# Fireflies-17/Speech-Inpainting

Hardware: AMD Instinct MI355X
Metric: real-time factor (audio-sec/wall-sec) per GPU, 4 s clips @16 kHz, 200 ms mask (higher is better)
Workload: dtype encoder GEMMs and attention products: bf16 MFMA, fp32 accumulate (softmax, LayerNorm, head, arg-max in fp32); vocoder: fp16 MFMA (operands rounded to fp16, saturating), fp32 accumulate, activations stored as fp16; 1 GPU; BASELINE configs[1]: batch=32 x 4 s clips per GPU, 200 ms mask, HuBERT-base + HiFi-GAN V1; step = masked log-mel front-end -> encoder -> arg-max/splice -> vocoder on resident raw clips; global_batch=32, clip_samples=64000, mask_frames=10, parallelism=utterance-sharded x1

## Files before the change

### include/si_hip.h

```cpp
#ifndef SI_HIP_H
#define SI_HIP_H

#include <stddef.h>
#include <stdint.h>

#ifdef __cplusplus
extern "C" {
#endif

#define SI_ABI_VERSION 3

enum {
    SI_OK = 0,
    SI_EINVAL = -1,
    SI_ENOMEM = -2,
    SI_EHIP = -3,
    SI_ESTATE = -4,
    SI_EWEIGHTS = -5
};

enum {
    SI_MATH_F32 = 0,
    SI_MATH_BF16 = 1,
    SI_MATH_BF16X3 = 2,
// ... 241 lines not shown
typedef struct si_profile_entry {
    char name[48];
    int32_t launches;
    int32_t reserved;
    double ms;
    double flops;
    double bytes;
} si_profile_entry;
int si_profile_start(si_ctx* ctx, int max_launches);
int si_profile_filter(si_ctx* ctx, const char* family);
int si_profile_stop(si_ctx* ctx, si_profile_entry* out, int capacity, int* count);

int si_debug_capture(si_ctx* ctx, const char* name, float* dst, long capacity);
long si_debug_size(si_ctx* ctx, const char* name);

#ifdef __cplusplus
}
#endif
#endif
```

### speech_inpainting_amd/csrc/api.hip

```cpp
#include <cmath>
#include <cstdarg>
#include <cstdio>
#include <cstdlib>
#include <cstring>
#include <map>
#include <sstream>
#include <string>
#include <vector>

#include "common.h"

namespace {

struct HostTensor {
    const float* data = nullptr;
    std::vector<long> shape;
    long numel() const { long n = 1; for (long d : shape) n *= d; return n; }
};

struct GemmW {
    size_t w = 0, w_lo = 0, bias = 0;
    int Cin = 0, N = 0, Npad = 0, ntaps = 0, groups = 1, math = 0;
    bool has_bias = false;
};
// ... 33 lines not shown
    std::string prof_filter;
    std::vector<std::string> prof_names;
    std::vector<ProfRec> prof_recs;
    std::vector<hipEvent_t> prof_pool;
    size_t prof_used = 0;
    int prof_open = -1;
    int num_cus = 0;
    std::map<const void*, size_t> dyn_lds;
    bool opt_voc_opready = true, opt_voc_res16 = true, opt_enc_opready = true, opt_att_bf16 = true, opt_enc_lingemm = true;
    bool opt_enc_posconv = true;
    int opt_ln_fuse = 1;
    int opt_voc_upsgemm = 1;
    int opt_ffn_pad = 64;
    int opt_gemmcu = 1;
    int opt_voc_chain = 1;
    int opt_voc_fuse = 1;
    char* fe_dev = nullptr;
    size_t fe_dft = 0, fe_hann = 0, fe_basis = 0, fe_lo = 0, fe_hi = 0;
    std::vector<int32_t> vl_host;
    static constexpr int VL_SLOTS = 4;
    int32_t* vl_pin[VL_SLOTS] = {nullptr, nullptr, nullptr, nullptr};
    size_t vl_pin_ints[VL_SLOTS] = {0, 0, 0, 0};
    hipEvent_t vl_ev[VL_SLOTS] = {nullptr, nullptr, nullptr, nullptr};
    int vl_next = 0;
    float* km_cnorm = nullptr;
    int km_cnorm_cap = 0;
};

static char g_create_err[512] = "";

// ... 486 lines not shown
    EncDims e = enc_dims(d, N);
    size_t cmax = 0;
    for (int i = 0; i < d.num_conv; ++i) cmax = std::max(cmax, (size_t)e.L[i + 1] * d.conv_dim[i]);
    const size_t BT = (size_t)B * std::max(e.T, 1);
    size_t f = 2 * (size_t)B * cmax + BT * d.conv_dim[d.num_conv - 1] + BT * d.hidden_size * 3 + BT * 3 * d.hidden_size + BT * d.intermediate_size +
               (size_t)B * d.conv_dim[0] * 2 + BT * 2;
    const size_t h16 = (BT * d.conv_dim[d.num_conv - 1] + 2 * BT * d.hidden_size + BT * (d.intermediate_size + 128)) * 2;
    return f * 4 + h16 + (size_t)B * 16 + (size_t)B * 4 + si_conv0_partials_bytes(B, N) + 41 * 256 +
           align_up((size_t)(SI_MAX_CONV + 3) * (B + 1) * 4, 256);
}

int vocoder_chunk(const si_model_desc& d, int B) { int c = d.vocoder_chunk > 0 ? d.vocoder_chunk : 32; return std::min(c, std::max(B, 1)); }

long voc_tout(int Tm, int stretch) { return stretch ? (long)std::floor((double)Tm * (441.0 / 256.0)) : Tm; }

size_t vocoder_ws_bytes(const si_ctx* ctx, int B, int Tm, int stretch) {
    const si_model_desc& d = ctx->d;
    const int Bc = vocoder_chunk(d, B);
    const long Tout = voc_tout(Tm, stretch);
    size_t lc_max = (size_t)Tout * d.up_initial_channel;
    long L = Tout; int c = d.up_initial_channel;
    for (int i = 0; i < d.num_ups; ++i) { L *= d.up_rates[i]; c = stage_channels(ctx, i); lc_max = std::max(lc_max, (size_t)L * c); }
    const size_t f = (size_t)Bc * Tout * ctx->lay.mel_ld + 9 * (size_t)Bc * lc_max;
    return f * 4 + 32 * 256 + align_up((size_t)(2 * SI_MAX_UPS + 3) * B * 4, 256);
}

TapGemmParams gemm_params(const si_ctx* ctx, const GemmW& G) {
    TapGemmParams p{};
    p.w = ctx->wdev + G.w;
    p.w_lo = G.math == SI_MATH_BF16X3 ? ctx->wdev + G.w_lo : nullptr;
    p.bias = G.has_bias ? reinterpret_cast<const float*>(ctx->wdev + G.bias) : nullptr;
    p.Cin = G.Cin; p.N = G.N; p.Npad = G.Npad; p.ntaps = G.ntaps; p.groups = G.groups;
    p.stride = 1; p.dil = 1; p.pad = 0; p.pro_slope = 1.f; p.act = SI_ACT_NONE; p.alpha = 1.f; p.accumulate = 0;
    p.out16_slope = 1.f;
    p.nseg = 1;
    return p;
}

struct UpsGeom { int u, pad; long Lout; int M; };
// ... 56 lines not shown
    if (!out) return si_fail(nullptr, SI_EINVAL, "si_create: out is NULL");
    *out = nullptr;
    int rc = check_desc(nullptr, desc);
    if (rc) return rc;
    int ndev = 0;
    if (hipGetDeviceCount(&ndev) != hipSuccess || device_id < 0 || device_id >= ndev)
        return si_fail(nullptr, SI_EHIP, "si_create: device %d not available (%d HIP devices visible)", device_id, ndev);
    si_ctx* ctx = new si_ctx();
    ctx->device = device_id;
    ctx->d = *desc;
    auto env_flag = [](const char* name) { const char* v = getenv(name); return v ? atoi(v) != 0 : true; };
    ctx->opt_voc_opready = env_flag("SI_VOC_OPREADY");
    ctx->opt_voc_res16 = env_flag("SI_VOC_RES16");
    ctx->opt_voc_fuse = getenv("SI_VOC_FUSE") ? atoi(getenv("SI_VOC_FUSE")) : 1;
    ctx->opt_voc_chain = getenv("SI_VOC_CHAIN") ? atoi(getenv("SI_VOC_CHAIN")) : 1;
    ctx->opt_enc_opready = env_flag("SI_ENC_OPREADY");
    ctx->opt_att_bf16 = env_flag("SI_ATT_BF16");
    ctx->opt_enc_lingemm = env_flag("SI_ENC_LINGEMM");
    ctx->opt_enc_posconv = env_flag("SI_ENC_POSCONV");
    ctx->opt_gemmcu = getenv("SI_ENC_GEMMCU") ? atoi(getenv("SI_ENC_GEMMCU")) : 1;
    ctx->opt_ln_fuse = getenv("SI_ENC_LNFUSE") ? atoi(getenv("SI_ENC_LNFUSE")) : 1;
    ctx->opt_voc_upsgemm = getenv("SI_VOC_UPSGEMM") ? atoi(getenv("SI_VOC_UPSGEMM")) : 1;
    ctx->opt_ffn_pad = getenv("SI_ENC_FFNPAD") ? std::min(128, std::max(0, atoi(getenv("SI_ENC_FFNPAD")) / 8 * 8)) : 64;
    plan_layout(ctx);
    *out = ctx;
    return SI_OK;
}

void si_destroy(si_ctx* ctx) {
    if (!ctx) return;
// ... 688 lines not shown
                    const UpsGeom g = ups_geom(d, i, Lb);
                    t[(size_t)(2 + i) * B + b] = (int32_t)g.Lout;
                    t[(size_t)(2 + d.num_ups + i) * B + b] = g.M;
                    Lb = g.Lout;
                }
            }
            return SI_OK;
        })) return trc;
        SI_HIP_CHECK(hipMemsetAsync(wav_out, 0, (size_t)B * Lwav * sizeof(float), st));
    }
    float* ext_ws = W.floats((size_t)Bc_max * Tout * Ly.mel_ld);
    float* buf_ws[6];
    unsigned short* h16_ws[6];
    for (auto& b : buf_ws) b = W.floats((size_t)Bc_max * lc_max);
    for (auto& b : h16_ws) b = reinterpret_cast<unsigned short*>(W.bytes((size_t)Bc_max * lc_max * 2));
    const bool opr = ctx->opt_voc_opready && (d.vocoder_math == SI_MATH_BF16 || d.vocoder_math == SI_MATH_F16);
    const bool r16 = opr && ctx->opt_voc_res16 && d.vocoder_math == SI_MATH_F16;
    const int fuse_mask = ctx->opt_voc_fuse == 1 ? ~0 : ctx->opt_voc_fuse;
    if (!W.ok) return si_fail(ctx, SI_ENOMEM, "internal: vocoder workspace carve exceeded its own estimate");
    const int nk = d.num_rb;
    static const char* upn[] = {"ups0", "ups1", "ups2", "ups3", "ups4", "ups5", "ups6", "ups7"};
    static const char* stn[] = {"stage0", "stage1", "stage2", "stage3", "stage4", "stage5", "stage6", "stage7"};

    auto run = [&](int b0, int Bc, float* ext, float* const* buf, unsigned short* const* h16, hipStream_t st) -> int {
        int rc;
        auto tap16 = [&](const void* src, long n, const char* fmt, int a = 0, int b = 0, int c = 0) -> int {
            return (r16 && !ctx->dbg_capture.empty()) ? si_tap(ctx, st, {src, n, 2}, fmt, a, b, c) : SI_OK;
        };
        auto tap32 = [&](TapSrc s, const char* fmt, int a = 0, int b = 0, int c = 0) -> int {
            return (!r16 && !ctx->dbg_capture.empty()) ? si_tap(ctx, st, s, fmt, a, b, c) : SI_OK;
        };
        const int32_t* dTm = vl ? tab.dev + b0 : nullptr;
        auto dLs = [&](int sidx) -> const int32_t* { return vl ? tab.dev + (size_t)(1 + sidx) * B + b0 : nullptr; };
        auto hLs = [&](int sidx) -> const int32_t* { return vl ? tab.host + (size_t)(1 + sidx) * B + b0 : nullptr; };
        auto rows_of = [&](const int32_t* h, long uniform) { if (!h) return (double)Bc * uniform; double r = 0; for (int b = 0; b < Bc; ++b) r += h[b]; return r; };
        auto stage_conv = [&](const GemmW& G, int sidx, long L, int ld_in, int cin, int dil) {
            TapGemmParams p = gemm_params(ctx, G);
            p.nseg = Bc; p.Lin = (int)L; p.M = (int)L; p.ldx = ld_in; p.x_seg_stride = L * ld_in;
            p.dil = dil; p.pad = dil * (G.ntaps - 1) / 2; p.ldo = G.N; p.o_seg_stride = L * G.N; p.olimit = p.o_seg_stride;
// ... 54 lines not shown
                p.pro_slope = act_in ? 1.f : in_slope;
                const int urc = act_in ? si_launch_gemmcu_tc(ctx, p, st, true) : 1;
                if (urc < 0) return urc;
                if (urc > 0 && (rc = si_launch_tapgemm(ctx, G.math, p, st))) return rc;
            }
            const long nst = (long)Bc * Lo * cout;
            if (!r16 && (rc = si_tap(ctx, st, {U, nst}, upn[i]))) return rc;
            if ((rc = tap16(U16, nst, "ups%d.f16", i))) return rc;
            const bool act_next = ups_takes_activated(i + 1, Lo, cout);
            struct BlockOut { float alpha; int accumulate; bool copy16; float slope16; };
            auto block_out = [&](int j, bool last) {
                const bool completes = last && j == nk - 1;
                return BlockOut{last ? 1.0f / nk : 1.f, last && j > 0, r16 || !last || (completes && i + 1 < d.num_ups),
                                (r16 && !(completes && act_next)) ? 1.f : 0.1f};
            };
            for (int j = 0; j < nk; ++j) {
                const ResW& R = Ly.rbs[(size_t)i * nk + j];
                const int rk = d.rb_kernels[j];
                const float* y = U;
                const unsigned short* y16 = U16;
                const BlockOut whole = block_out(j, true);
                if (r16 && d.resblock_type != 2 && (fuse_mask & cout) && ctx->opt_voc_chain && d.num_dil == 3 && whole.slope16 == 1.f) {
                    ResChainParams cp{};
                    cp.y16 = U16; cp.out16 = xs16; cp.B = Bc; cp.L = (int)Lo; cp.k = rk; cp.alpha = whole.alpha; cp.accumulate = whole.accumulate;
                    cp.lens = dLs(i + 1); cp.lens_host = hLs(i + 1);
                    for (int n = 0; n < 3; ++n) {
                        const TapGemmParams w1 = gemm_params(ctx, R.c1[n]), w2 = gemm_params(ctx, R.c2[n]);
                        cp.w1[n] = static_cast<const unsigned short*>(w1.w); cp.w2[n] = static_cast<const unsigned short*>(w2.w);
                        cp.b1[n] = w1.bias; cp.b2[n] = w2.bias; cp.dil[n] = d.rb_dilations[j][n];
                    }
                    const int crc = si_launch_reschain(ctx, cout, cp, st);
                    if (crc < 0) return crc;
                    if (crc == 0) {
                        if ((rc = tap16(xs16, nst, "stage%d.rb%d.p%d.f16", i, j, d.num_dil - 1))) return rc;
                        continue;
                    }
                }
                for (int n = 0; n < d.num_dil; ++n) {
                    const int dl = d.rb_dilations[j][n];
                    const bool last = (n == d.num_dil - 1);
                    float* ynext = last ? xs : buf[4 + (n & 1)];
                    unsigned short* ynext16 = last ? xs16 : h16[4 + (n & 1)];
                    const BlockOut o = block_out(j, last);
                    auto residual_conv = [&](const GemmW& G, int dil, float slope, const float* in, const unsigned short* in16) {
                        TapGemmParams q = stage_conv(G, i + 1, Lo, cout, cout, dil);
                        q.x = in; q.out = ynext; q.res = y; q.pro_slope = slope;
                        if (opr) {
                            q.x = nullptr; q.x16 = in16;
                            if (r16) { q.res = nullptr; q.res16 = y16; q.out = nullptr; }
                            if (o.copy16) { q.out16 = ynext16; q.out16_slope = o.slope16; }
                        }
                        q.alpha = o.alpha; q.accumulate = o.accumulate; q.acc16 = r16 && o.accumulate;
                        return si_launch_tapgemm(ctx, G.math, q, st);
                    };
                    if (d.resblock_type == 2) {
                        if ((rc = residual_conv(R.c1[n], dl, in_slope, y, y16))) return rc;
                    } else {
// ... 21 lines not shown
                    y16 = ynext16;
                }
            }
            if (!r16 && (rc = si_tap(ctx, st, {xs, nst}, stn[i]))) return rc;
            if ((rc = tap16(xs16, nst, "stage%d.f16", i))) return rc;
            std::swap(x, xs);
            std::swap(x16, xs16);
            Lc = Lo; c = cout; act_in = act_next;
        }
        return si_launch_conv_post(ctx, x, wf(ctx, Ly.post_w), wf(ctx, Ly.post_b), Bc, (int)Lc, c, 7, wav_out + (size_t)b0 * Lwav, st,
                                   r16 ? x16 : nullptr, dLs(d.num_ups), hLs(d.num_ups));
    };

    for (int b0 = 0; b0 < B; b0 += Bc_max) {
        const int Bc = std::min(Bc_max, B - b0);
        if (int rc = run(b0, Bc, ext_ws, buf_ws, h16_ws, st)) return rc;
    }
    return SI_OK;
}

}

namespace {

constexpr int FE_NFFT = 1024, FE_HOP = 441, FE_PAD = 312, FE_NMEL = 80, FE_SR = 22050, FE_NBIN = FE_NFFT / 2 + 1;
constexpr double FE_FMIN = 0.0, FE_FMAX = 8000.0;
constexpr int FE_KC = 528, FE_KS = 512;
constexpr int FE_FRAME = FE_KC + FE_KS;
constexpr int FE_IMOFF = 516;
constexpr int FE_LDSPEC = 1032;

// ... 387 lines not shown
```

### speech_inpainting_amd/csrc/common.h

```cpp
#pragma once
#include <hip/hip_runtime.h>
#include <stdint.h>

#include "../../include/si_hip.h"

#define SI_HIP_CHECK(expr)                                                                      \
    do {                                                                                        \
        hipError_t _e = (expr);                                                                 \
        if (_e != hipSuccess) return si_fail_hip(ctx, _e, #expr, __FILE__, __LINE__);           \
    } while (0)

int si_fail_hip(si_ctx* ctx, hipError_t e, const char* what, const char* file, int line);
int si_fail(si_ctx* ctx, int code, const char* fmt, ...);
void si_prof_begin(si_ctx* ctx, const char* name, double flops, double bytes, hipStream_t st);
void si_prof_end(si_ctx* ctx, hipStream_t st);
const char* si_prof_shape_name(const char* name, long M, int N, int K);
int si_ensure_dyn_lds(si_ctx* ctx, const void* kern, size_t bytes);
int si_num_cus(si_ctx* ctx);

typedef unsigned short bf16_t;

struct SiVlTile { int b, row0, L; };
#ifdef __HIPCC__
__device__ __forceinline__ SiVlTile si_vl_tile(const int32_t* __restrict__ lens, int B, int step, int t) {
// ... 236 lines not shown

struct UpsampleParams {
    const unsigned short* x16;
    const unsigned short* w;
    const float* bias;
    unsigned short* out16;
    int B, Lin, M;
    int Cin, N, taps;
    long ooff;
    long o_clip_stride, o_clip_elems;
    const int32_t* lens_lin; const int32_t* lens_m; const int32_t* lens_m_host;
    int total_tiles;
};
int si_launch_upsample_stream(si_ctx* ctx, const UpsampleParams& p, hipStream_t st);

struct ResPairParams {
    const unsigned short* y16;
    unsigned short* out16;
    const unsigned short* w1;
    const unsigned short* w2;
    const float* b1;
    const float* b2;
    int B, L, k, dil;
    float alpha;
    int accumulate;
    const int32_t* lens; const int32_t* lens_host;
    int total_tiles;
    float out_slope;
};
int si_launch_respair_wide(si_ctx* ctx, int C, const ResPairParams& p, hipStream_t st);
struct ResChainParams {
    const unsigned short* y16;
    unsigned short* out16;
    const unsigned short* w1[3];
    const unsigned short* w2[3];
    const float* b1[3];
    const float* b2[3];
    int B, L, k;
    int dil[3];
    float alpha;
    int accumulate;
    const int32_t* lens; const int32_t* lens_host;
    int total_tiles;
};
int si_launch_reschain(si_ctx* ctx, int C, const ResChainParams& p, hipStream_t st);
// ... 17 lines not shown
```

### speech_inpainting_amd/csrc/respair_wide.hip

```cpp
#include <algorithm>
#include <cstdio>
#include <cstdlib>

#include "common.h"

typedef float f32x4 __attribute__((ext_vector_type(4)));
typedef unsigned int u32x4 __attribute__((ext_vector_type(4)));
typedef unsigned int u32x2 __attribute__((ext_vector_type(2)));
typedef _Float16 f16x8 __attribute__((ext_vector_type(8)));
typedef _Float16 f16x4 __attribute__((ext_vector_type(4)));

template <int ROWB>
__device__ __forceinline__ int swz16(int row) {
    if constexpr (ROWB >= 256) return (row & 7) << 5;
    else return ((row >> 1) & 3) << 5;
}

#ifdef RPW_TIMELINE
__device__ unsigned long long rpw_tl[2][10];
#define RPW_TL_DECL unsigned long long tl_t = wall_clock64(); unsigned long long tl_acc[6] = {0, 0, 0, 0, 0, 0}; unsigned long long tl_tiles = 0; unsigned long long tl_w = 0, tl_sub[2] = {0, 0};
#define RPW_TL_W0 tl_w = wall_clock64();
#define RPW_TL_W1(q) tl_sub[q] += wall_clock64() - tl_w;
#define RPW_TL(ph) { const unsigned long long n_ = wall_clock64(); tl_acc[ph] += n_ - tl_t; tl_t = n_; }
#define RPW_TL_TILE ++tl_tiles;
// ... 25 lines not shown
    constexpr int CPRY = C / 8, CPRW = BKW / 8;
    constexpr int NCH = C / BKW;
    constexpr int KS = BKW / 32;
    constexpr int YBYTES = (R1 + RPW_HALO) * ROWBY;
    constexpr int WBYTES = C * ROWBW;
    constexpr int WSLOTS = C * CPRW / NT;
    constexpr int YSLOTS = ((R1 + RPW_HALO) * CPRY + NT - 1) / NT;
    constexpr int YRPP = NT / CPRY, WRPP = NT / CPRW;
    static_assert(C * CPRW % NT == 0 && NT % CPRY == 0 && NT % CPRW == 0, "staging maps");
    static_assert(R1 * ROWBO <= YBYTES + 2 * WBYTES, "the output image reuses the operand region (not the biases behind it)");

    __builtin_amdgcn_s_setreg((0 << 11) | (23 << 6) | 1, 1);
    extern __shared__ __attribute__((aligned(16))) char smem[];
    char* const Ys = smem;
    char* const Ws = smem + YBYTES;
    float* const Bs = reinterpret_cast<float*>(smem + YBYTES + 2 * WBYTES);

    const int tid = threadIdx.x, lane = tid & 63, wave = tid >> 6;
    const int r16 = lane & 15, kg = lane >> 4;
    const int wm0 = (wave / WARPS_N) * 64, wn0 = (wave % WARPS_N) * 64;
    const int k = p.k, d = p.dil;
    const int p1 = d * (k - 1) / 2, p2 = (k - 1) / 2;
    const int BMo = R1 - (k - 1);
    const int R0 = R1 + (k - 1) * d;
    const int tiles_x = (p.L + BMo - 1) / BMo;
    const int total = VL ? p.total_tiles : tiles_x * p.B;
    auto tile_of = [&](int t, int& tb, int& tm0, int& tL) {
        if constexpr (VL) { const SiVlTile v = si_vl_tile(p.lens, p.B, BMo, t); tb = v.b; tm0 = v.row0; tL = v.L; }
        else { tb = t / tiles_x; tm0 = (t - tb * tiles_x) * BMo; tL = p.L; }
    };
    const __amdgpu_buffer_rsrc_t w1rsrc = __builtin_amdgcn_make_buffer_rsrc(const_cast<unsigned short*>(p.w1), 0, k * C * C * 2, 0x00020000);
    const __amdgpu_buffer_rsrc_t w2rsrc = __builtin_amdgcn_make_buffer_rsrc(const_cast<unsigned short*>(p.w2), 0, k * C * C * 2, 0x00020000);

    const int NS1 = k * NCH, NS = 2 * NS1;
    const int wc = tid % CPRW, wr0 = tid / CPRW;
    u32x4 rw[WSLOTS];
    auto issueW1 = [&](int s, int i) {
        const bool second = s >= NS1;
        const int q = second ? s - NS1 : s;
        const int tap = q / NCH, ch = q - tap * NCH;
        const int soff = __builtin_amdgcn_readfirstlane((tap * C * C + ch * BKW) * 2);
        const int n = wr0 + i * WRPP;
        rw[i] = __builtin_amdgcn_raw_buffer_load_b128(second ? w2rsrc : w1rsrc, (n * C + 8 * wc) * 2, soff, 0);
    };
    auto issueW = [&](int s) {
#pragma unroll
        for (int i = 0; i < WSLOTS; ++i) issueW1(s, i);
    };
    auto storeW1 = [&](char* dst, int i) {
        const int n = wr0 + i * WRPP;
        *reinterpret_cast<u32x4*>(dst + n * ROWBW + ((wc << 4) ^ swz16<ROWBW>(n))) = rw[i];
    };
    auto storeW = [&](char* dst) {
#pragma unroll
        for (int i = 0; i < WSLOTS; ++i) storeW1(dst, i);
    };
    const int yc = tid % CPRY, yr0 = tid / CPRY;
    u32x4 ry[YSLOTS];
    auto issueY = [&](int t) {
        int tb, tm0, tL;
        tile_of(t, tb, tm0, tL);
        const int trow0 = tm0 - p2 - p1;
        const __amdgpu_buffer_rsrc_t rs = __builtin_amdgcn_make_buffer_rsrc(const_cast<unsigned short*>(p.y16 + (long)tb * p.L * C), 0, tL * C * 2, 0x00020000);
#pragma unroll
        for (int i = 0; i < YSLOTS; ++i)
            ry[i] = __builtin_amdgcn_raw_buffer_load_b128(rs, ((trow0 + yr0 + i * YRPP) * C + 8 * yc) * 2, 0, 0);
    };

    if (tid < C / 2) {
        const int which = tid / (C / 4), c4 = (tid % (C / 4)) * 4;
        *reinterpret_cast<f32x4*>(Bs + which * C + c4) = *reinterpret_cast<const f32x4*>((which ? p.b2 : p.b1) + c4);
    }
    const int preW = (wn0 + r16) * ROWBW + (swz16<ROWBW>(wn0 + r16) ^ (kg << 4));
    issueW(0);
    issueY(blockIdx.x);
    RPW_TL_DECL

  for (int tile = blockIdx.x; tile < total; tile += gridDim.x) {
    const int nxt = tile + (int)gridDim.x < total ? tile + (int)gridDim.x : tile;
    int b, m0, Lb;
    tile_of(tile, b, m0, Lb);
    const int t_row0 = m0 - p2;
    const long seg = (long)b * p.L * C;
    const __amdgpu_buffer_rsrc_t yrsrc = __builtin_amdgcn_make_buffer_rsrc(const_cast<unsigned short*>(p.y16 + seg), 0, Lb * C * 2, 0x00020000);
    const __amdgpu_buffer_rsrc_t orsrc = __builtin_amdgcn_make_buffer_rsrc(p.out16 + seg, 0, Lb * C * 2, 0x00020000);

    storeW(Ws);
    issueW(1);
#pragma unroll
    for (int i = 0; i < YSLOTS; ++i) {
        const int r = yr0 + i * YRPP;
        if ((i + 1) * YRPP <= R1 || r < R0) {
            f16x8 h = __builtin_bit_cast(f16x8, ry[i]);
            h = __builtin_elementwise_max(h, h * (_Float16)0.1f);
            *reinterpret_cast<f16x8*>(Ys + r * ROWBY + ((yc << 4) ^ swz16<ROWBY>(r))) = h;
        }
    }
    __syncthreads();
    RPW_TL(0)

// ... 83 lines not shown
#pragma unroll
                    for (int q = 0; q < 2; ++q) {
                        const auto r = __builtin_amdgcn_permlane16_swap(pk[0][q], pk[1][q], false, false);
                        pk[0][q] = r[0]; pk[1][q] = r[1];
                    }
                    const int ch = ((wn0 + 16 * j) >> 3) + (kg >> 1);
                    *reinterpret_cast<u32x4*>(Ys + ms * ROWBY + ((ch << 4) ^ swz16<ROWBY>(ms))) = u32x4{pk[0][0], pk[0][1], pk[1][0], pk[1][1]};
                }
            }
            init_acc(Bs + C);
            RPW_TL(2)
        }
        if (++ch == NCH) { ch = 0; if (++tap == k) tap = 0; }
        __syncthreads();
    }
    if constexpr (!ACC) issueY(nxt);
    __builtin_amdgcn_sched_barrier(0);
    compute(tap, ch * (BKW * 2), Ws + ((NS - 1) & 1) * WBYTES, [](int) {});
    RPW_TL(3)
    constexpr int ORPP = NT / CPRY;
    constexpr int OPASS = R1 / ORPP;
    const int c8 = tid % CPRY, or0 = tid / CPRY;
    u32x4 res[OPASS], prev[ACC ? OPASS : 1];
    int goff[OPASS];
#pragma unroll
    for (int it = 0; it < OPASS; ++it) {
        const int o = or0 + it * ORPP;
        const int grow = m0 + o;
        goff[it] = (o < BMo && grow < Lb) ? (grow * C + 8 * c8) * 2 : (int)0x80000000;
        res[it] = __builtin_amdgcn_raw_buffer_load_b128(yrsrc, goff[it], 0, 0);
        if constexpr (ACC) prev[it] = __builtin_amdgcn_raw_buffer_load_b128(orsrc, goff[it], 0, 0);
// ... 3 lines not shown
    RPW_TL_W1(0)
    RPW_TL_W0

#pragma unroll
    for (int i = 0; i < 4; ++i) {
        const int m = wm0 + 16 * i + r16;
#pragma unroll
        for (int j = 0; j < 4; ++j) {
            const int co = ((wn0 + 16 * j) >> 2) + kg;
            *reinterpret_cast<f32x4*>(smem + m * ROWBO + ((co ^ (m & 15)) << 4)) = acc[i][j];
        }
    }
    RPW_TL_W1(1)
    __syncthreads();
    RPW_TL(4)
    issueW(0);
    {
        const bool oact = p.out_slope != 0.f && p.out_slope != 1.f;
#pragma unroll
        for (int it = 0; it < OPASS; ++it) {
            const int o = or0 + it * ORPP;
            const f32x4 a0 = *reinterpret_cast<const f32x4*>(smem + o * ROWBO + (((2 * c8) ^ (o & 15)) << 4));
            const f32x4 a1 = *reinterpret_cast<const f32x4*>(smem + o * ROWBO + (((2 * c8 + 1) ^ (o & 15)) << 4));
            const f16x8 rh = __builtin_bit_cast(f16x8, res[it]);
            f16x8 ph = {};
            if constexpr (ACC) ph = __builtin_bit_cast(f16x8, prev[it]);
            f16x8 out;
#pragma unroll
            for (int e = 0; e < 8; ++e) {
                const float a = e < 4 ? a0[e] : a1[e - 4];
                float v = (a + (float)rh[e]) * p.alpha;
                if constexpr (ACC) v += (float)ph[e];
                if (oact) v = v > 0.f ? v : v * p.out_slope;
                out[e] = (_Float16)v;
            }
            __builtin_amdgcn_raw_buffer_store_b128(__builtin_bit_cast(u32x4, out), orsrc, goff[it], 0, 0);
        }
    }
    if constexpr (ACC) issueY(nxt);
    __syncthreads();
    RPW_TL(5)
    RPW_TL_TILE
  }
  RPW_TL_FLUSH
}

template <int C, int R1, int WARPS_M, int WARPS_N, int BKW>
static int respair_wide_launch(si_ctx* ctx, const ResPairParams& p0, hipStream_t st) {
    const ResPairParams& p = p0;
    const int BMo = R1 - (p.k - 1);
    const size_t lds = (size_t)(R1 + RPW_HALO) * C * 2 + 2 * (size_t)C * BKW * 2 + 2 * (size_t)C * 4;
    const bool vl = p0.lens != nullptr;
    auto kern = vl ? (p.accumulate ? respair_wide_kernel<C, R1, WARPS_M, WARPS_N, BKW, true, true> : respair_wide_kernel<C, R1, WARPS_M, WARPS_N, BKW, false, true>)
                   : (p.accumulate ? respair_wide_kernel<C, R1, WARPS_M, WARPS_N, BKW, true, false> : respair_wide_kernel<C, R1, WARPS_M, WARPS_N, BKW, false, false>);
    if (int rc = si_ensure_dyn_lds(ctx, reinterpret_cast<const void*>(kern), lds)) return rc;
    const int total = vl ? (int)si_vl_tiles(p.lens_host, p.B, BMo) : ((p.L + BMo - 1) / BMo) * p.B;
    if (total <= 0) return SI_OK;
    ResPairParams pk = p0;
    pk.total_tiles = total;
    const int grid = std::min(total, si_num_cus(ctx) * (WARPS_M * WARPS_N == 4 ? 2 : 1));
    char name[48];
    snprintf(name, sizeof(name), p.accumulate ? "respair_f16_c%d_acc" : "respair_f16_c%d", C);
    double rows = (double)p.B * p.L;
    if (vl) { rows = 0; for (int b = 0; b < p.B; ++b) rows += p.lens_host[b]; }
    const double elems = rows * C;
    si_prof_begin(ctx, name, 2.0 * 2.0 * elems * C * p.k, elems * (2.0 + 2.0 + (p.accumulate ? 2.0 : 0.0)) + 2.0 * 2.0 * p.k * C * C, st);
    hipLaunchKernelGGL(kern, dim3(grid), dim3(64 * WARPS_M * WARPS_N), lds, st, pk);
    si_prof_end(ctx, st);
    SI_HIP_CHECK(hipGetLastError());
    return SI_OK;
}

int si_launch_respair_wide(si_ctx* ctx, int C, const ResPairParams& p, hipStream_t st) {
    if (C == 128) return respair_wide_launch<128, 256, 4, 2, 128>(ctx, p, st);
    if (C == 256) return respair_wide_launch<256, 128, 2, 4, 64>(ctx, p, st);
    return 1;
}
```

### speech_inpainting_amd/native.py

```python
from __future__ import annotations

import ctypes as C
import os
from typing import Optional

import numpy as np
import torch

from .arch import HubertArch, VocoderArch

_HERE = os.path.dirname(os.path.abspath(__file__))
LIB_PATH = os.environ.get("SI_HIP_LIB") or os.path.join(_HERE, "libsi_hip.so")

SI_MATH = {"fp32": 0, "f32": 0, "bf16": 1, "bf16x3": 2, "fp16": 3, "f16": 3}
SI_MAX_CONV, SI_MAX_UPS, SI_MAX_RB, SI_MAX_DIL = 8, 8, 4, 4

EXPORTS = ["si_version", "si_create", "si_destroy", "si_last_error", "si_load_weights", "si_alloc_weights",
           "si_weights_device_ptr", "si_weights_check", "si_workspace_bytes", "si_hubert_forward", "si_hubert_forward_padded", "si_hubert_forward_varlen", "si_hubert_extract_features", "si_code_splice", "si_codebook_splice",
           "si_codebook_splice_varlen", "si_hifigan_forward_varlen", "si_mel_frontend_varlen",
           "si_codebook_splice_labels", "si_codebook_metrics", "si_kmeans_assign", "si_mel_metrics", "si_sisdr", "si_unit_frontend",
           "si_f0_encoder_weight_floats", "si_f0_encoder_frames", "si_f0_encoder_workspace_bytes", "si_f0_encoder_forward",
           "si_resample_poly", "si_resample_sinc", "si_pcm16", "si_extend_mel", "si_hifigan_forward", "si_mel_frames", "si_mel_workspace_bytes", "si_mel_frontend", "si_num_frames",
           "si_vocoder_samples", "si_profile_start", "si_profile_filter", "si_profile_stop",
           "si_debug_capture", "si_debug_size",
           "si_hubert_forward_spans", "si_mel_frontend_spans", "si_codebook_splice_spans", "si_codebook_splice_labels_spans",
           "si_codebook_metrics_spans", "si_wave_peak", "si_gather_windows", "si_patch_compose",
           "si_cut_clips", "si_patch_regions"]
SI_MAX_SPANS = 16


class _F0EncStruct(C.Structure):
    _fields_ = [(n, C.c_int32) for n in ("in_width", "out_width", "width", "n_state", "depth", "down_t", "stride_t", "dilation_growth")]


class F0EncDesc:

    def __init__(self, in_width=1, out_width=128, width=32, depth=4, down_t=4, stride_t=2, dilation_growth=3, m_conv=1.0):
        self.in_width, self.out_width, self.width, self.depth = int(in_width), int(out_width), int(width), int(depth)
        self.down_t, self.stride_t, self.dilation_growth = int(down_t), int(stride_t), int(dilation_growth)
        self.n_state = int(m_conv * width)

    def as_struct(self) -> _F0EncStruct:
# ... 233 lines not shown
    lib.si_extend_mel.argtypes = [vp, vp, i32, i32, vp, vp]
    lib.si_hifigan_forward.argtypes = [vp, vp, i32, i32, i32, vp, vp, sz, vp]
    lib.si_mel_frames.argtypes = [i32]
    lib.si_mel_workspace_bytes.argtypes = [vp, i32, i32, C.POINTER(sz)]
    lib.si_mel_frontend.argtypes = [vp, vp, vp, vp, i32, i32, i32, vp, vp, sz, vp]
    lib.si_hubert_forward_spans.argtypes = [vp, vp, C.POINTER(SpanTableStruct), vp, i32, i32, i32, vp, vp, sz, vp]
    lib.si_mel_frontend_spans.argtypes = [vp, vp, C.POINTER(SpanTableStruct), vp, i32, i32, i32, vp, vp, sz, vp]
    lib.si_codebook_splice_spans.argtypes = [vp, vp, i32, i32, vp, vp, i32, vp, i32, vp, vp]
    lib.si_codebook_splice_labels_spans.argtypes = [vp, vp, i32, vp, vp, i32, vp, i32, vp]
    lib.si_codebook_metrics_spans.argtypes = [vp, vp, i32, i32, vp, vp, i32, vp, vp, vp, vp, vp, vp]
    lib.si_wave_peak.argtypes = [vp, vp, C.POINTER(SpanTableStruct), vp, i32, i32, vp, vp]
    lib.si_gather_windows.argtypes = [vp, vp, i32, i32, vp, vp, i32, i32, vp, vp]
    lib.si_patch_compose.argtypes = [vp, vp, C.POINTER(SpanTableStruct), vp, C.POINTER(PatchTableStruct), vp, i32, vp, i32, i32, vp, vp, vp]
    lib.si_cut_clips.argtypes = [vp, vp, i32, vp, vp, i32, i32, vp, vp]
    lib.si_patch_regions.argtypes = [vp, vp, i32, C.POINTER(RegionTableStruct), vp, i32, vp, vp, vp, vp]
    lib.si_num_frames.argtypes = [vp, i32]
    lib.si_vocoder_samples.argtypes = [vp, i32, i32]
    lib.si_debug_capture.argtypes = [vp, C.c_char_p, vp, C.c_long]
    lib.si_debug_size.argtypes = [vp, C.c_char_p]
    lib.si_debug_size.restype = C.c_long
    lib.si_profile_start.argtypes = [vp, i32]
    lib.si_profile_filter.argtypes = [vp, C.c_char_p]
    lib.si_profile_stop.argtypes = [vp, C.POINTER(ProfileEntry), i32, C.POINTER(i32)]
    for name in EXPORTS:
        if name not in ("si_destroy", "si_last_error", "si_debug_size"):
            getattr(lib, name).restype = i32
    if path is None:
        _lib = lib
    return lib

# ... 504 lines not shown
```

Measured before the change: 11310 x real-time (audio-sec/wall-sec); `value` = whole-job aggregate over n_gpus, `value_per_gpu` = the per-GPU figure the metric names.

## Merge the three resblock branch conv pairs into one multi-job vocoder launch

```diff
diff --git a/include/si_hip.h b/include/si_hip.h
--- a/include/si_hip.h
+++ b/include/si_hip.h
@@ -279,6 +279,9 @@
 int si_debug_capture(si_ctx* ctx, const char* name, float* dst, long capacity);
 long si_debug_size(si_ctx* ctx, const char* name);
 
+int si_respair_tile_plan(int C, int B, int L, const int32_t* lens, const int32_t* ks, int njobs, int32_t* tile0, int32_t* job_of,
+                         int32_t* tile_of, int cap);
+
 #ifdef __cplusplus
 }
 #endif
diff --git a/speech_inpainting_amd/csrc/api.hip b/speech_inpainting_amd/csrc/api.hip
--- a/speech_inpainting_amd/csrc/api.hip
+++ b/speech_inpainting_amd/csrc/api.hip
@@ -1,3 +1,4 @@
+#include <algorithm>
 #include <cmath>
 #include <cstdarg>
 #include <cstdio>
@@ -71,6 +72,7 @@
     int opt_ffn_pad = 64;
     int opt_gemmcu = 1;
     int opt_voc_chain = 1;
+    int opt_voc_merge = 1;
     int opt_voc_fuse = 1;
     char* fe_dev = nullptr;
     size_t fe_dft = 0, fe_hann = 0, fe_basis = 0, fe_lo = 0, fe_hi = 0;
@@ -587,6 +589,20 @@
 
 long voc_tout(int Tm, int stretch) { return stretch ? (long)std::floor((double)Tm * (441.0 / 256.0)) : Tm; }
 
+bool stage_merges(const si_ctx* ctx, int i) {
+    const si_model_desc& d = ctx->d;
+    const bool r16 = ctx->opt_voc_opready && ctx->opt_voc_res16 && d.vocoder_math == SI_MATH_F16;
+    const int cout = stage_channels(ctx, i);
+    const int fuse_mask = ctx->opt_voc_fuse == 1 ? ~0 : ctx->opt_voc_fuse;
+    return ctx->opt_voc_merge && r16 && d.resblock_type != 2 && d.num_rb == 3 && d.num_dil == 3 && (cout == 128 || cout == 256) && (fuse_mask & cout);
+}
+size_t vocoder_merge_elems(const si_ctx* ctx, long Tout) {
+    size_t m = 0;
+    long L = Tout;
+    for (int i = 0; i < ctx->d.num_ups; ++i) { L *= ctx->d.up_rates[i]; if (stage_merges(ctx, i)) m = std::max(m, (size_t)L * stage_channels(ctx, i)); }
+    return m;
+}
+
 size_t vocoder_ws_bytes(const si_ctx* ctx, int B, int Tm, int stretch) {
     const si_model_desc& d = ctx->d;
     const int Bc = vocoder_chunk(d, B);
@@ -594,8 +610,8 @@
     size_t lc_max = (size_t)Tout * d.up_initial_channel;
     long L = Tout; int c = d.up_initial_channel;
     for (int i = 0; i < d.num_ups; ++i) { L *= d.up_rates[i]; c = stage_channels(ctx, i); lc_max = std::max(lc_max, (size_t)L * c); }
-    const size_t f = (size_t)Bc * Tout * ctx->lay.mel_ld + 9 * (size_t)Bc * lc_max;
-    return f * 4 + 32 * 256 + align_up((size_t)(2 * SI_MAX_UPS + 3) * B * 4, 256);
+    const size_t f = (size_t)Bc * Tout * ctx->lay.mel_ld + 9 * (size_t)Bc * lc_max + 2 * (size_t)Bc * vocoder_merge_elems(ctx, Tout);
+    return f * 4 + 36 * 256 + align_up((size_t)(2 * SI_MAX_UPS + 3) * B * 4, 256);
 }
 
 TapGemmParams gemm_params(const si_ctx* ctx, const GemmW& G) {
@@ -682,6 +698,7 @@
     ctx->opt_voc_res16 = env_flag("SI_VOC_RES16");
     ctx->opt_voc_fuse = getenv("SI_VOC_FUSE") ? atoi(getenv("SI_VOC_FUSE")) : 1;
     ctx->opt_voc_chain = getenv("SI_VOC_CHAIN") ? atoi(getenv("SI_VOC_CHAIN")) : 1;
+    ctx->opt_voc_merge = getenv("SI_VOC_MERGE") ? atoi(getenv("SI_VOC_MERGE")) : 1;
     ctx->opt_enc_opready = env_flag("SI_ENC_OPREADY");
     ctx->opt_att_bf16 = env_flag("SI_ATT_BF16");
     ctx->opt_enc_lingemm = env_flag("SI_ENC_LINGEMM");
@@ -1400,6 +1417,8 @@
     unsigned short* h16_ws[6];
     for (auto& b : buf_ws) b = W.floats((size_t)Bc_max * lc_max);
     for (auto& b : h16_ws) b = reinterpret_cast<unsigned short*>(W.bytes((size_t)Bc_max * lc_max * 2));
+    unsigned short* mrg_ws[4] = {};
+    if (const size_t me = vocoder_merge_elems(ctx, Tout)) for (auto& b : mrg_ws) b = reinterpret_cast<unsigned short*>(W.bytes((size_t)Bc_max * me * 2));
     const bool opr = ctx->opt_voc_opready && (d.vocoder_math == SI_MATH_BF16 || d.vocoder_math == SI_MATH_F16);
     const bool r16 = opr && ctx->opt_voc_res16 && d.vocoder_math == SI_MATH_F16;
     const int fuse_mask = ctx->opt_voc_fuse == 1 ? ~0 : ctx->opt_voc_fuse;
@@ -1408,7 +1427,7 @@
     static const char* upn[] = {"ups0", "ups1", "ups2", "ups3", "ups4", "ups5", "ups6", "ups7"};
     static const char* stn[] = {"stage0", "stage1", "stage2", "stage3", "stage4", "stage5", "stage6", "stage7"};
 
-    auto run = [&](int b0, int Bc, float* ext, float* const* buf, unsigned short* const* h16, hipStream_t st) -> int {
+    auto run = [&](int b0, int Bc, float* ext, float* const* buf, unsigned short* const* h16, unsigned short* const* mrg, hipStream_t st) -> int {
         int rc;
         auto tap16 = [&](const void* src, long n, const char* fmt, int a = 0, int b = 0, int c = 0) -> int {
             return (r16 && !ctx->dbg_capture.empty()) ? si_tap(ctx, st, {src, n, 2}, fmt, a, b, c) : SI_OK;
@@ -1493,13 +1512,36 @@
                 return BlockOut{last ? 1.0f / nk : 1.f, last && j > 0, r16 || !last || (completes && i + 1 < d.num_ups),
                                 (r16 && !(completes && act_next)) ? 1.f : 0.1f};
             };
+            int merged = 0;
+            unsigned short* const own16[3][2] = {{h16[4], h16[5]}, {mrg[0], mrg[1]}, {mrg[2], mrg[3]}};
+            if (stage_merges(ctx, i)) {
+                int ord[3] = {0, 1, 2};
+                std::stable_sort(ord, ord + 3, [&](int a, int b) { return d.rb_kernels[a] > d.rb_kernels[b]; });
+                for (int n = 0; n < 2; ++n) {
+                    ResPairParams mp{};
+                    mp.B = Bc; mp.L = (int)Lo; mp.lens = dLs(i + 1); mp.lens_host = hLs(i + 1); mp.njobs = 3;
+                    for (int q = 0; q < 3; ++q) {
+                        const int j = ord[q];
+                        const ResW& R = Ly.rbs[(size_t)i * nk + j];
+                        const TapGemmParams w1 = gemm_params(ctx, R.c1[n]), w2 = gemm_params(ctx, R.c2[n]);
+                        const BlockOut o = block_out(j, false);
+                        mp.job[q] = ResPairJob{n ? own16[j][0] : U16, own16[j][n], static_cast<const unsigned short*>(w1.w), static_cast<const unsigned short*>(w2.w),
+                                               w1.bias, w2.bias, d.rb_kernels[j], d.rb_dilations[j][n], o.alpha, o.slope16, 0, 0};
+                    }
+                    const int mrc = si_launch_respair_merged(ctx, cout, mp, st);
+                    if (mrc < 0) return mrc;
+                    if (mrc > 0) break;
+                    merged = n + 1;
+                    for (int j = 0; j < 3; ++j) if ((rc = tap16(own16[j][n], nst, "stage%d.rb%d.p%d.f16", i, j, n))) return rc;
+                }
+            }
             for (int j = 0; j < nk; ++j) {
                 const ResW& R = Ly.rbs[(size_t)i * nk + j];
                 const int rk = d.rb_kernels[j];
                 const float* y = U;
-                const unsigned short* y16 = U16;
+                const unsigned short* y16 = merged ? own16[j][merged - 1] : U16;
                 const BlockOut whole = block_out(j, true);
-                if (r16 && d.resblock_type != 2 && (fuse_mask & cout) && ctx->opt_voc_chain && d.num_dil == 3 && whole.slope16 == 1.f) {
+                if (!merged && r16 && d.resblock_type != 2 && (fuse_mask & cout) && ctx->opt_voc_chain && d.num_dil == 3 && whole.slope16 == 1.f) {
                     ResChainParams cp{};
                     cp.y16 = U16; cp.out16 = xs16; cp.B = Bc; cp.L = (int)Lo; cp.k = rk; cp.alpha = whole.alpha; cp.accumulate = whole.accumulate;
                     cp.lens = dLs(i + 1); cp.lens_host = hLs(i + 1);
@@ -1515,11 +1557,11 @@
                         continue;
                     }
                 }
-                for (int n = 0; n < d.num_dil; ++n) {
+                for (int n = merged; n < d.num_dil; ++n) {
                     const int dl = d.rb_dilations[j][n];
                     const bool last = (n == d.num_dil - 1);
                     float* ynext = last ? xs : buf[4 + (n & 1)];
-                    unsigned short* ynext16 = last ? xs16 : h16[4 + (n & 1)];
+                    unsigned short* ynext16 = last ? xs16 : merged ? own16[j][n & 1] : h16[4 + (n & 1)];
                     const BlockOut o = block_out(j, last);
                     auto residual_conv = [&](const GemmW& G, int dil, float slope, const float* in, const unsigned short* in16) {
                         TapGemmParams q = stage_conv(G, i + 1, Lo, cout, cout, dil);
@@ -1571,7 +1613,7 @@
 
     for (int b0 = 0; b0 < B; b0 += Bc_max) {
         const int Bc = std::min(Bc_max, B - b0);
-        if (int rc = run(b0, Bc, ext_ws, buf_ws, h16_ws, st)) return rc;
+        if (int rc = run(b0, Bc, ext_ws, buf_ws, h16_ws, mrg_ws, st)) return rc;
     }
     return SI_OK;
 }
diff --git a/speech_inpainting_amd/csrc/common.h b/speech_inpainting_amd/csrc/common.h
--- a/speech_inpainting_amd/csrc/common.h
+++ b/speech_inpainting_amd/csrc/common.h
@@ -274,6 +274,25 @@
 };
 int si_launch_upsample_stream(si_ctx* ctx, const UpsampleParams& p, hipStream_t st);
 
+constexpr int SI_RESPAIR_JOBS = 3;
+struct ResPairJob {
+    const unsigned short* y16;
+    unsigned short* out16;
+    const unsigned short* w1;
+    const unsigned short* w2;
+    const float* b1;
+    const float* b2;
+    int k, dil;
+    float alpha, out_slope;
+    int tile0;
+    int tiles_x;
+};
+#ifdef __HIPCC__
+__host__ __device__
+#endif
+inline int si_respair_job_of(int t, int tile0_1, int tile0_2) { return (t >= tile0_1) + (t >= tile0_2); }
+long si_respair_plan(const int* ks, int njobs, int R1, int B, int L, const int32_t* lens_host, int* tile0, int* tiles_x);
+
 struct ResPairParams {
     const unsigned short* y16;
     unsigned short* out16;
@@ -287,8 +306,11 @@
     const int32_t* lens; const int32_t* lens_host;
     int total_tiles;
     float out_slope;
+    int njobs;
+    ResPairJob job[SI_RESPAIR_JOBS];
 };
 int si_launch_respair_wide(si_ctx* ctx, int C, const ResPairParams& p, hipStream_t st);
+int si_launch_respair_merged(si_ctx* ctx, int C, const ResPairParams& p, hipStream_t st);
 struct ResChainParams {
     const unsigned short* y16;
     unsigned short* out16;
diff --git a/speech_inpainting_amd/csrc/respair_wide.hip b/speech_inpainting_amd/csrc/respair_wide.hip
--- a/speech_inpainting_amd/csrc/respair_wide.hip
+++ b/speech_inpainting_amd/csrc/respair_wide.hip
@@ -63,25 +63,40 @@
     extern __shared__ __attribute__((aligned(16))) char smem[];
     char* const Ys = smem;
     char* const Ws = smem + YBYTES;
-    float* const Bs = reinterpret_cast<float*>(smem + YBYTES + 2 * WBYTES);
 
     const int tid = threadIdx.x, lane = tid & 63, wave = tid >> 6;
     const int r16 = lane & 15, kg = lane >> 4;
     const int wm0 = (wave / WARPS_N) * 64, wn0 = (wave % WARPS_N) * 64;
-    const int k = p.k, d = p.dil;
-    const int p1 = d * (k - 1) / 2, p2 = (k - 1) / 2;
-    const int BMo = R1 - (k - 1);
-    const int R0 = R1 + (k - 1) * d;
-    const int tiles_x = (p.L + BMo - 1) / BMo;
-    const int total = VL ? p.total_tiles : tiles_x * p.B;
-    auto tile_of = [&](int t, int& tb, int& tm0, int& tL) {
-        if constexpr (VL) { const SiVlTile v = si_vl_tile(p.lens, p.B, BMo, t); tb = v.b; tm0 = v.row0; tL = v.L; }
-        else { tb = t / tiles_x; tm0 = (t - tb * tiles_x) * BMo; tL = p.L; }
-    };
-    const __amdgpu_buffer_rsrc_t w1rsrc = __builtin_amdgcn_make_buffer_rsrc(const_cast<unsigned short*>(p.w1), 0, k * C * C * 2, 0x00020000);
-    const __amdgpu_buffer_rsrc_t w2rsrc = __builtin_amdgcn_make_buffer_rsrc(const_cast<unsigned short*>(p.w2), 0, k * C * C * 2, 0x00020000);
-
-    const int NS1 = k * NCH, NS = 2 * NS1;
+    const int total = p.total_tiles;
+    auto job_of = [&](int t) { return ACC ? 0 : si_respair_job_of(t, p.job[1].tile0, p.job[2].tile0); };
+    auto tile_of = [&](int t, int j, int& tb, int& tm0, int& tL) {
+        const int bmo = R1 - (p.job[j].k - 1), tl = t - p.job[j].tile0;
+        if constexpr (VL) {
+            const SiVlTile v = si_vl_tile(p.lens, p.B, bmo, tl);
+            tb = __builtin_amdgcn_readfirstlane(v.b); tm0 = __builtin_amdgcn_readfirstlane(v.row0); tL = __builtin_amdgcn_readfirstlane(v.L);
+        }
+        else { const int tiles_x = p.job[j].tiles_x; tb = tl / tiles_x; tm0 = (tl - tb * tiles_x) * bmo; tL = p.L; }
+    };
+    int job, k, d, p2, BMo, R0;
+    int NS1, NS;
+    __amdgpu_buffer_rsrc_t w1rsrc, w2rsrc;
+    float* const Bs = reinterpret_cast<float*>(smem + YBYTES + 2 * WBYTES);
+    auto set_job = [&](int j) {
+        job = j;
+        k = p.job[j].k; d = p.job[j].dil;
+        p2 = (k - 1) / 2;
+        BMo = R1 - (k - 1);
+        R0 = R1 + (k - 1) * d;
+        NS1 = k * NCH; NS = 2 * NS1;
+        w1rsrc = __builtin_amdgcn_make_buffer_rsrc(const_cast<unsigned short*>(p.job[j].w1), 0, k * C * C * 2, 0x00020000);
+        w2rsrc = __builtin_amdgcn_make_buffer_rsrc(const_cast<unsigned short*>(p.job[j].w2), 0, k * C * C * 2, 0x00020000);
+        if (threadIdx.x < C / 2) {
+            const int which = threadIdx.x / (C / 4), c4 = (threadIdx.x % (C / 4)) * 4;
+            *reinterpret_cast<f32x4*>(Bs + which * C + c4) = *reinterpret_cast<const f32x4*>((which ? p.job[j].b2 : p.job[j].b1) + c4);
+        }
+    };
+    set_job(job_of(blockIdx.x));
+
     const int wc = tid % CPRW, wr0 = tid / CPRW;
     u32x4 rw[WSLOTS];
     auto issueW1 = [&](int s, int i) {
@@ -96,6 +111,11 @@
 #pragma unroll
         for (int i = 0; i < WSLOTS; ++i) issueW1(s, i);
     };
+    auto issueW0 = [&](int j) {
+        const __amdgpu_buffer_rsrc_t rs = __builtin_amdgcn_make_buffer_rsrc(const_cast<unsigned short*>(p.job[j].w1), 0, p.job[j].k * C * C * 2, 0x00020000);
+#pragma unroll
+        for (int i = 0; i < WSLOTS; ++i) rw[i] = __builtin_amdgcn_raw_buffer_load_b128(rs, ((wr0 + i * WRPP) * C + 8 * wc) * 2, 0, 0);
+    };
     auto storeW1 = [&](char* dst, int i) {
         const int n = wr0 + i * WRPP;
         *reinterpret_cast<u32x4*>(dst + n * ROWBW + ((wc << 4) ^ swz16<ROWBW>(n))) = rw[i];
@@ -106,33 +126,31 @@
     };
     const int yc = tid % CPRY, yr0 = tid / CPRY;
     u32x4 ry[YSLOTS];
-    auto issueY = [&](int t) {
-        int tb, tm0, tL;
-        tile_of(t, tb, tm0, tL);
-        const int trow0 = tm0 - p2 - p1;
-        const __amdgpu_buffer_rsrc_t rs = __builtin_amdgcn_make_buffer_rsrc(const_cast<unsigned short*>(p.y16 + (long)tb * p.L * C), 0, tL * C * 2, 0x00020000);
+    auto issueY = [&](int j, int tb, int tm0, int tL) {
+        const int jk = p.job[j].k;
+        const int trow0 = tm0 - (jk - 1) / 2 - p.job[j].dil * (jk - 1) / 2;
+        const __amdgpu_buffer_rsrc_t rs = __builtin_amdgcn_make_buffer_rsrc(const_cast<unsigned short*>(p.job[j].y16 + (long)tb * p.L * C), 0, tL * C * 2, 0x00020000);
 #pragma unroll
         for (int i = 0; i < YSLOTS; ++i)
             ry[i] = __builtin_amdgcn_raw_buffer_load_b128(rs, ((trow0 + yr0 + i * YRPP) * C + 8 * yc) * 2, 0, 0);
     };
 
-    if (tid < C / 2) {
-        const int which = tid / (C / 4), c4 = (tid % (C / 4)) * 4;
-        *reinterpret_cast<f32x4*>(Bs + which * C + c4) = *reinterpret_cast<const f32x4*>((which ? p.b2 : p.b1) + c4);
-    }
     const int preW = (wn0 + r16) * ROWBW + (swz16<ROWBW>(wn0 + r16) ^ (kg << 4));
-    issueW(0);
-    issueY(blockIdx.x);
+    issueW0(job);
+    int b, m0, Lb;
+    tile_of(blockIdx.x, job, b, m0, Lb);
+    issueY(job, b, m0, Lb);
     RPW_TL_DECL
 
   for (int tile = blockIdx.x; tile < total; tile += gridDim.x) {
     const int nxt = tile + (int)gridDim.x < total ? tile + (int)gridDim.x : tile;
-    int b, m0, Lb;
-    tile_of(tile, b, m0, Lb);
+    const int njob = job_of(nxt);
+    int nb, nm0, nLb;
+    if constexpr (!ACC) tile_of(nxt, njob, nb, nm0, nLb);
     const int t_row0 = m0 - p2;
     const long seg = (long)b * p.L * C;
-    const __amdgpu_buffer_rsrc_t yrsrc = __builtin_amdgcn_make_buffer_rsrc(const_cast<unsigned short*>(p.y16 + seg), 0, Lb * C * 2, 0x00020000);
-    const __amdgpu_buffer_rsrc_t orsrc = __builtin_amdgcn_make_buffer_rsrc(p.out16 + seg, 0, Lb * C * 2, 0x00020000);
+    const __amdgpu_buffer_rsrc_t yrsrc = __builtin_amdgcn_make_buffer_rsrc(const_cast<unsigned short*>(p.job[job].y16 + seg), 0, Lb * C * 2, 0x00020000);
+    const __amdgpu_buffer_rsrc_t orsrc = __builtin_amdgcn_make_buffer_rsrc(p.job[job].out16 + seg, 0, Lb * C * 2, 0x00020000);
 
     storeW(Ws);
     issueW(1);
@@ -246,7 +264,7 @@
         if (++ch == NCH) { ch = 0; if (++tap == k) tap = 0; }
         __syncthreads();
     }
-    if constexpr (!ACC) issueY(nxt);
+    if constexpr (!ACC) issueY(njob, nb, nm0, nLb);
     __builtin_amdgcn_sched_barrier(0);
     compute(tap, ch * (BKW * 2), Ws + ((NS - 1) & 1) * WBYTES, [](int) {});
     RPW_TL(3)
@@ -280,9 +298,10 @@
     RPW_TL_W1(1)
     __syncthreads();
     RPW_TL(4)
-    issueW(0);
+    issueW0(njob);
     {
-        const bool oact = p.out_slope != 0.f && p.out_slope != 1.f;
+        const float alpha = p.job[job].alpha, out_slope = p.job[job].out_slope;
+        const bool oact = out_slope != 0.f && out_slope != 1.f;
 #pragma unroll
         for (int it = 0; it < OPASS; ++it) {
             const int o = or0 + it * ORPP;
@@ -295,15 +314,17 @@
 #pragma unroll
             for (int e = 0; e < 8; ++e) {
                 const float a = e < 4 ? a0[e] : a1[e - 4];
-                float v = (a + (float)rh[e]) * p.alpha;
+                float v = (a + (float)rh[e]) * alpha;
                 if constexpr (ACC) v += (float)ph[e];
-                if (oact) v = v > 0.f ? v : v * p.out_slope;
+                if (oact) v = v > 0.f ? v : v * out_slope;
                 out[e] = (_Float16)v;
             }
             __builtin_amdgcn_raw_buffer_store_b128(__builtin_bit_cast(u32x4, out), orsrc, goff[it], 0, 0);
         }
     }
-    if constexpr (ACC) issueY(nxt);
+    if constexpr (ACC) { tile_of(nxt, njob, nb, nm0, nLb); issueY(njob, nb, nm0, nLb); }
+    if (njob != job) set_job(njob);
+    b = nb; m0 = nm0; Lb = nLb;
     __syncthreads();
     RPW_TL(5)
     RPW_TL_TILE
@@ -311,26 +332,53 @@
   RPW_TL_FLUSH
 }
 
+long si_respair_plan(const int* ks, int njobs, int R1, int B, int L, const int32_t* lens_host, int* tile0, int* tiles_x) {
+    long total = 0;
+    for (int j = 0; j < SI_RESPAIR_JOBS; ++j) {
+        tile0[j] = 0x7fffffff; tiles_x[j] = 0;
+        if (j >= njobs) continue;
+        if (j > 0 && ks[j] > ks[j - 1]) return -1;
+        const int BMo = R1 - (ks[j] - 1);
+        tile0[j] = (int)total;
+        tiles_x[j] = (L + BMo - 1) / BMo;
+        total += lens_host ? si_vl_tiles(lens_host, B, BMo) : (long)tiles_x[j] * B;
+    }
+    return total;
+}
+
 template <int C, int R1, int WARPS_M, int WARPS_N, int BKW>
-static int respair_wide_launch(si_ctx* ctx, const ResPairParams& p0, hipStream_t st) {
-    const ResPairParams& p = p0;
-    const int BMo = R1 - (p.k - 1);
+static int respair_wide_launch(si_ctx* ctx, const ResPairParams& p, hipStream_t st) {
     const size_t lds = (size_t)(R1 + RPW_HALO) * C * 2 + 2 * (size_t)C * BKW * 2 + 2 * (size_t)C * 4;
-    const bool vl = p0.lens != nullptr;
+    const bool vl = p.lens != nullptr;
     auto kern = vl ? (p.accumulate ? respair_wide_kernel<C, R1, WARPS_M, WARPS_N, BKW, true, true> : respair_wide_kernel<C, R1, WARPS_M, WARPS_N, BKW, false, true>)
                    : (p.accumulate ? respair_wide_kernel<C, R1, WARPS_M, WARPS_N, BKW, true, false> : respair_wide_kernel<C, R1, WARPS_M, WARPS_N, BKW, false, false>);
     if (int rc = si_ensure_dyn_lds(ctx, reinterpret_cast<const void*>(kern), lds)) return rc;
-    const int total = vl ? (int)si_vl_tiles(p.lens_host, p.B, BMo) : ((p.L + BMo - 1) / BMo) * p.B;
-    if (total <= 0) return SI_OK;
-    ResPairParams pk = p0;
-    pk.total_tiles = total;
-    const int grid = std::min(total, si_num_cus(ctx) * (WARPS_M * WARPS_N == 4 ? 2 : 1));
+    ResPairParams pk = p;
+    if (p.njobs == 0) {
+        pk.njobs = 1;
+        pk.job[0] = ResPairJob{p.y16, p.out16, p.w1, p.w2, p.b1, p.b2, p.k, p.dil, p.alpha, p.out_slope, 0, 0};
+    }
+    if (pk.njobs < 1 || pk.njobs > SI_RESPAIR_JOBS || (pk.njobs > 1 && p.accumulate)) return si_fail(ctx, SI_EINVAL, "respair: %d jobs in one launch", pk.njobs);
+    for (int j = pk.njobs; j < SI_RESPAIR_JOBS; ++j) pk.job[j] = pk.job[0];
+    int ks[SI_RESPAIR_JOBS] = {}, tile0[SI_RESPAIR_JOBS], tiles_x[SI_RESPAIR_JOBS];
+    for (int j = 0; j < pk.njobs; ++j) ks[j] = pk.job[j].k;
+    const long total = si_respair_plan(ks, pk.njobs, R1, p.B, p.L, p.lens_host, tile0, tiles_x);
+    if (total < 0 || total > 0x7ffffffe) return si_fail(ctx, SI_EINVAL, "respair: jobs must come in descending k, %ld tiles", total);
+    if (total == 0) return SI_OK;
+    for (int j = 0; j < SI_RESPAIR_JOBS; ++j) { pk.job[j].tile0 = tile0[j]; pk.job[j].tiles_x = tiles_x[j]; }
+    pk.total_tiles = (int)total;
+    const int grid = (int)std::min<long>(total, si_num_cus(ctx) * (WARPS_M * WARPS_N == 4 ? 2 : 1));
     char name[48];
-    snprintf(name, sizeof(name), p.accumulate ? "respair_f16_c%d_acc" : "respair_f16_c%d", C);
+    snprintf(name, sizeof(name), pk.njobs > 1 ? "respair_f16_c%d_x%d" : p.accumulate ? "respair_f16_c%d_acc" : "respair_f16_c%d", C, pk.njobs);
     double rows = (double)p.B * p.L;
     if (vl) { rows = 0; for (int b = 0; b < p.B; ++b) rows += p.lens_host[b]; }
     const double elems = rows * C;
-    si_prof_begin(ctx, name, 2.0 * 2.0 * elems * C * p.k, elems * (2.0 + 2.0 + (p.accumulate ? 2.0 : 0.0)) + 2.0 * 2.0 * p.k * C * C, st);
+    double flops = 0, bytes = 0;
+    for (int j = 0; j < pk.njobs; ++j) {
+        flops += 2.0 * 2.0 * elems * C * ks[j];
+        bytes += elems * (2.0 + 2.0 + (p.accumulate ? 2.0 : 0.0)) + 2.0 * 2.0 * ks[j] * C * C;
+    }
+    si_prof_begin(ctx, name, flops, bytes, st);
     hipLaunchKernelGGL(kern, dim3(grid), dim3(64 * WARPS_M * WARPS_N), lds, st, pk);
     si_prof_end(ctx, st);
     SI_HIP_CHECK(hipGetLastError());
@@ -342,3 +390,28 @@
     if (C == 256) return respair_wide_launch<256, 128, 2, 4, 64>(ctx, p, st);
     return 1;
 }
+
+int si_launch_respair_merged(si_ctx* ctx, int C, const ResPairParams& p, hipStream_t st) {
+    if ((C != 128 && C != 256) || p.njobs < 2 || p.njobs > SI_RESPAIR_JOBS || p.accumulate || ((long)p.L + 1024) * C * 2 >= (1L << 31)) return 1;
+    for (int j = 0; j < p.njobs; ++j) {
+        const ResPairJob& q = p.job[j];
+        if (q.k < 3 || q.k > 11 || (q.k & 1) == 0 || (q.k - 1) * q.dil > 50 || !q.b1 || !q.b2 || (j > 0 && q.k > p.job[j - 1].k)) return 1;
+    }
+    if ((p.lens == nullptr) != (p.lens_host == nullptr)) return si_fail(ctx, SI_EINVAL, "respair: ragged batches need the lengths on the device and on the host");
+    return si_launch_respair_wide(ctx, C, p, st);
+}
+
+extern "C" int si_respair_tile_plan(int C, int B, int L, const int32_t* lens, const int32_t* ks, int njobs, int32_t* tile0, int32_t* job_of, int32_t* tile_of, int cap) {
+    if ((C != 128 && C != 256) || njobs < 1 || njobs > SI_RESPAIR_JOBS || B < 1 || L < 1 || !ks || !tile0) return SI_EINVAL;
+    int k[SI_RESPAIR_JOBS] = {}, t0[SI_RESPAIR_JOBS], tx[SI_RESPAIR_JOBS];
+    for (int j = 0; j < njobs; ++j) { if (ks[j] < 3 || ks[j] > 11 || !(ks[j] & 1)) return SI_EINVAL; k[j] = ks[j]; }
+    const long total = si_respair_plan(k, njobs, C == 128 ? 256 : 128, B, L, lens, t0, tx);
+    if (total < 0 || total > 0x7ffffffe) return SI_EINVAL;
+    for (int j = 0; j < njobs; ++j) tile0[j] = t0[j];
+    tile0[njobs] = (int32_t)total;
+    for (long t = 0; t < total && t < cap && job_of && tile_of; ++t) {
+        const int j = si_respair_job_of((int)t, t0[1], t0[2]);
+        job_of[t] = j; tile_of[t] = (int32_t)t - t0[j];
+    }
+    return SI_OK;
+}
diff --git a/speech_inpainting_amd/native.py b/speech_inpainting_amd/native.py
--- a/speech_inpainting_amd/native.py
+++ b/speech_inpainting_amd/native.py
@@ -25,7 +25,7 @@
            "si_debug_capture", "si_debug_size",
            "si_hubert_forward_spans", "si_mel_frontend_spans", "si_codebook_splice_spans", "si_codebook_splice_labels_spans",
            "si_codebook_metrics_spans", "si_wave_peak", "si_gather_windows", "si_patch_compose",
-           "si_cut_clips", "si_patch_regions"]
+           "si_cut_clips", "si_patch_regions", "si_respair_tile_plan"]
 SI_MAX_SPANS = 16
 
 
@@ -289,6 +289,7 @@
     lib.si_patch_compose.argtypes = [vp, vp, C.POINTER(SpanTableStruct), vp, C.POINTER(PatchTableStruct), vp, i32, vp, i32, i32, vp, vp, vp]
     lib.si_cut_clips.argtypes = [vp, vp, i32, vp, vp, i32, i32, vp, vp]
     lib.si_patch_regions.argtypes = [vp, vp, i32, C.POINTER(RegionTableStruct), vp, i32, vp, vp, vp, vp]
+    lib.si_respair_tile_plan.argtypes = [i32, i32, i32, vp, vp, i32, vp, vp, vp, i32]
     lib.si_num_frames.argtypes = [vp, i32]
     lib.si_vocoder_samples.argtypes = [vp, i32, i32]
     lib.si_debug_capture.argtypes = [vp, C.c_char_p, vp, C.c_long]
```

Result: faster. 11530 x real-time (audio-sec/wall-sec); `value` = whole-job aggregate over n_gpus, `value_per_gpu` = the per-GPU figure the metric names (median of 6 runs) (+1.9%).
